# nanoporetech/remora

Hardware: AMD Instinct MI355X
Metric: chunks/sec, 5mC CG ConvLSTM_w_ref inference (fused chunk arrays -> logits + label counts) (higher is better)
Workload: dtype f32; 1 GPU; synthetic 100-sig-pt CG chunks, ConvLSTM_w_ref size 64 k-mer (4,4) 2-class (BASELINE configs[2]), fp32

## Files before the change

remora_amd/csrc/k_lstm.hip:

```cpp
#include "rmr_internal.h"
#include "rmr_math.h"
#include "rmr_mma.h"

namespace rmr {

struct LstmArgs {
    const float *x;
    float *logits;
    const float *a_ih1, *a_hh1, *b1, *a_ih2, *b2, *w_fc, *b_fc;
    int64_t n;
    int T, num_out;
};

template <int KS, int G, int RS>
__device__ __forceinline__ void xproj(const float (&buf)[4][16][RS], int q, int nn,
                                      const float (&A)[4][KS], f32x4 (&acc)[4]) {
    const float *b = &buf[q][nn][0];
#pragma unroll
    for (int g = 0; g < G; ++g) {
        const f32x4 bx = *reinterpret_cast<const f32x4 *>(b + 4 * g);
#pragma unroll
        for (int j = 0; j < 4; ++j)
#pragma unroll
            for (int gt = 0; gt < 4; ++gt)
                acc[gt] = __builtin_amdgcn_mfma_f32_16x16x4f32(A[gt][g * 4 + j], bx[j], acc[gt], 0, 0, 0);
    }
}

__device__ __forceinline__ float fc_dot4(const f32x4 wv, const f32x4 y) {
    return fmaf(wv[3], y[3], fmaf(wv[2], y[2], fmaf(wv[1], y[1], wv[0] * y[0])));
}

__device__ __forceinline__ void gates(const f32x4 (&acc)[4], f32x4 &c, f32x4 &h) {
#pragma unroll
    for (int r = 0; r < 4; ++r) {
        const float ig = sigmoid_f(acc[0][r]), fg = sigmoid_f(acc[1][r]);
        const float gg = tanh_f(acc[2][r]), og = sigmoid_f(acc[3][r]);
        c[r] = fg * c[r] + ig * gg;
        h[r] = og * tanh_f(c[r]);
    }
}

template <int H, bool HAS_H, bool HAS_X, int ABL>
__device__ __forceinline__ void lstm_step(const float (&xb_img)[4][16][(H / 16 % 2 == 0) ? H / 4 + 4 : H / 4],
                                          const float (&hb_img)[4][16][(H / 16 % 2 == 0) ? H / 4 + 4 : H / 4],
                                          int q, int nn, const float (&Aih)[4][H / 4], const float (&Ahh)[4][H / 4],
                                          const f32x4 (&bias)[4], f32x4 (&acc)[4], f32x4 (&accN)[4], f32x4 &c, f32x4 &h) {
    constexpr int KS = H / 4, G = H / 16;
    constexpr int RS = (G % 2 == 0) ? H / 4 + 4 : H / 4;
    f32x4 bx[G];
    if (HAS_X) {
        const float *xb = &xb_img[q][nn][0];
#pragma unroll
        for (int g = 0; g < G; ++g) bx[g] = *reinterpret_cast<const f32x4 *>(xb + 4 * g);
    }
    if (HAS_H) xproj<KS, G, RS>(hb_img, q, nn, Ahh, acc);
#pragma unroll
    for (int gt = 0; gt < 4; ++gt) accN[gt] = bias[gt];
    float ig[4], fg[4], gg[4];
#pragma unroll
    for (int s = 0; s < KS; ++s) {
        __builtin_amdgcn_sched_barrier(0);
        if (HAS_X) {
#pragma unroll
            for (int gt = 0; gt < 4; ++gt)
                accN[gt] = __builtin_amdgcn_mfma_f32_16x16x4f32(Aih[gt][s], bx[s >> 2][s & 3], accN[gt], 0, 0, 0);
        }
        for (int piece = s * 16 / KS; piece < (s + 1) * 16 / KS; ++piece) {
            const int r = piece >> 2, st = piece & 3;
            if (ABL & 1) {
                if (st == 3) { c[r] += acc[0][r] * acc[1][r]; h[r] = acc[2][r] + acc[3][r] * c[r]; }
                continue;
            }
            if (st == 0) ig[r] = fast_rcp(1.0f + __builtin_amdgcn_exp2f(acc[0][r]));
            if (st == 1) fg[r] = fast_rcp(1.0f + __builtin_amdgcn_exp2f(acc[1][r]));
            if (st == 2) {
                gg[r] = fmaf(-2.0f, fast_rcp(1.0f + __builtin_amdgcn_exp2f(acc[2][r])), 1.0f);
                c[r] = fmaf(fg[r], c[r], ig[r] * gg[r]);
            }
            if (st == 3) {
                const float og = fast_rcp(1.0f + __builtin_amdgcn_exp2f(acc[3][r]));
                h[r] = og * tanh_f(c[r]);
            }
        }
    }
    __builtin_amdgcn_sched_barrier(0);
}

template <int H, int ABL = 0>
__global__ __launch_bounds__(4 * H, 2) void lstm_head_kernel(LstmArgs a) {
    constexpr int NW = H / 16;
    constexpr int KS = H / 4;
    constexpr int G = H / 16;
    constexpr int RS = (G % 2 == 0) ? H / 4 + 4 : H / 4;
    static_assert((16 * RS) % 64 == 0, "plane must be a multiple of 64 floats");
    __shared__ __attribute__((aligned(16))) float xbuf[2][4][16][RS];
    __shared__ __attribute__((aligned(16))) float hbuf[2][4][16][RS];
    __shared__ float part[NW][16][16];
    extern __shared__ __attribute__((aligned(16))) float w2_lds[];

    const int tid = threadIdx.x;
    const int lane = tid & 63, w = tid >> 6, q = lane >> 4, nn = lane & 15;
    float *const w2 = w2_lds + (size_t)w * 3 * KS * 64 + lane;
    {
        const float *src = a.a_ih2 + (size_t)w * 3 * KS * 64 + lane;
#pragma unroll 8
        for (int i = 0; i < 3 * KS; ++i) w2[i * 64] = src[(size_t)i * 64];
    }

    float Aih[4][KS], Ahh[4][KS];
#pragma unroll
    for (int gt = 0; gt < 4; ++gt) {
        const float *pi = a.a_ih1 + ((size_t)(w * 4 + gt) * KS) * 64 + lane;
        const float *ph = a.a_hh1 + ((size_t)(w * 4 + gt) * KS) * 64 + lane;
#pragma unroll
        for (int s = 0; s < KS; ++s) {
            Aih[gt][s] = pi[(size_t)s * 64];
            Ahh[gt][s] = ph[(size_t)s * 64];
        }
    }
    f32x4 bias[4];
#pragma unroll
    for (int gt = 0; gt < 4; ++gt)
        bias[gt] = *reinterpret_cast<const f32x4 *>(a.b1 + gt * H + 16 * w + 4 * q);

    const int st_row = tid / (H / 4), st_c4 = tid - st_row * (H / 4);
    const int st_q = st_c4 & 3, st_g = st_c4 >> 2;

    const int64_t n_groups = (a.n + 15) / 16;
    for (int64_t grp = blockIdx.x; grp < n_groups; grp += gridDim.x) {
        const int64_t chunk0 = grp * 16;
        int64_t st_chunk = chunk0 + st_row;
        if (st_chunk >= a.n) st_chunk = a.n - 1;
        const float4 *xsrc = reinterpret_cast<const float4 *>(a.x + (size_t)st_chunk * a.T * H) + st_c4;
        RMR_SYNC();
        *reinterpret_cast<float4 *>(&xbuf[0][st_q][st_row][4 * st_g]) = xsrc[0];
        *reinterpret_cast<float4 *>(&xbuf[1][st_q][st_row][4 * st_g]) = xsrc[(size_t)(a.T > 1 ? 1 : 0) * (H / 4)];
        RMR_SYNC();

        f32x4 c = {0.f, 0.f, 0.f, 0.f};
        f32x4 accA[4] = {bias[0], bias[1], bias[2], bias[3]}, accB[4];
        xproj<KS, G, RS>(xbuf[0], q, nn, Aih, accA);
        RMR_SYNC();
#define RMR_LSTM_STEP(HAS_H, HAS_X, t_, p_, in, out)                                                                   \
    do {                                                                                                               \
        const int tt = (t_), pp = (p_);                                                                                \
        const int tf = (tt + 2 < a.T) ? tt + 2 : a.T - 1;                                                              \
        const float4 xnext = xsrc[(size_t)tf * (H / 4)];                                                               \
        f32x4 h;                                                                                                       \
        lstm_step<H, HAS_H, HAS_X, ABL>(xbuf[pp ^ 1], hbuf[pp ^ 1], q, nn, Aih, Ahh, bias, in, out, c, h);             \
        *reinterpret_cast<f32x4 *>(&hbuf[pp][q][nn][4 * w]) = h;                                                       \
        *reinterpret_cast<float4 *>(&xbuf[pp][st_q][st_row][4 * st_g]) = xnext;                                        \
        if (!(ABL & 2)) RMR_SYNC();                           \
    } while (0)
        RMR_LSTM_STEP(false, true, 0, 0, accA, accB);
        int t = 1;
        for (; t + 2 < a.T; t += 2) {
            RMR_LSTM_STEP(true, true, t, 1, accB, accA);
            RMR_LSTM_STEP(true, true, t + 1, 0, accA, accB);
        }
        if (t + 1 < a.T) {
            RMR_LSTM_STEP(true, true, t, 1, accB, accA);
#pragma unroll
            for (int gt = 0; gt < 4; ++gt) accB[gt] = accA[gt];
            ++t;
        }
        if (t < a.T) RMR_LSTM_STEP(true, false, t, t & 1, accB, accA);
#undef RMR_LSTM_STEP

        f32x4 acc2[3];
#pragma unroll
        for (int gt = 0; gt < 3; ++gt)
            acc2[gt] = *reinterpret_cast<const f32x4 *>(a.b2 + gt * H + 16 * w + 4 * q);
        {
            const float *hb = &hbuf[(a.T - 1) & 1][q][nn][0];
#pragma unroll
            for (int g = 0; g < G; ++g) {
                f32x4 z = *reinterpret_cast<const f32x4 *>(hb + 4 * g);
#pragma unroll
                for (int j = 0; j < 4; ++j) z[j] = swish_f(z[j]);
#pragma unroll
                for (int j = 0; j < 4; ++j)
#pragma unroll
                    for (int gt = 0; gt < 3; ++gt) {
                        const float aw = w2[(gt * KS + g * 4 + j) * 64];
                        acc2[gt] = __builtin_amdgcn_mfma_f32_16x16x4f32(aw, z[j], acc2[gt], 0, 0, 0);
                    }
            }
        }
        f32x4 y;
#pragma unroll
        for (int r = 0; r < 4; ++r) {
            const float c2 = sigmoid_f(acc2[0][r]) * tanh_f(acc2[1][r]);
            const float h2 = sigmoid_f(acc2[2][r]) * tanh_f(c2);
            y[r] = swish_f(h2);
        }
        for (int o = 0; o < a.num_out; ++o) {
            const f32x4 wv = *reinterpret_cast<const f32x4 *>(a.w_fc + (size_t)o * H + 16 * w + 4 * q);
            float p = fc_dot4(wv, y);
            p += __shfl_xor(p, 16);
            p += __shfl_xor(p, 32);
            if (q == 0) part[w][nn][o] = p;
        }
        RMR_SYNC();
#pragma unroll
        for (int i0 = 0; i0 < 16 * 16; i0 += 4 * H) {
            const int i = i0 + tid;
            if (i < 16 * a.num_out) {
                const int ch = i / a.num_out, o = i - ch * a.num_out;
                if (chunk0 + ch < a.n) {
                    float s = a.b_fc[o];
#pragma unroll
                    for (int ww = 0; ww < NW; ++ww) s += part[ww][ch][o];
                    a.logits[(size_t)(chunk0 + ch) * a.num_out + o] = s;
                }
            }
        }
    }
}

struct LstmSmallArgs {
    const float *x;
    float *logits;
    const float *s_ih1, *s_hh1, *s_ih2;
    const float *b1, *b2, *w_fc, *b_fc;
    int64_t n;
    int T, num_out;
};

template <bool HAS_H, bool HAS_X>
__device__ __forceinline__ void small_step(const float (&Ahh)[64], const float (&Aih)[64], const float *hrow, const float *xrow, f32x4 &acc,
                                           f32x4 &accN) {
#pragma unroll
    for (int g = 0; g < 4; ++g) {
        f32x4 hv[4], xv[4];
#pragma unroll
        for (int qq = 0; qq < 4; ++qq) {
            if (HAS_H) hv[qq] = *reinterpret_cast<const f32x4 *>(hrow + 16 * g + 4 * qq);
            if (HAS_X) xv[qq] = *reinterpret_cast<const f32x4 *>(xrow + 16 * g + 4 * qq);
        }
#pragma unroll
        for (int j = 0; j < 4; ++j)
#pragma unroll
            for (int qq = 0; qq < 4; ++qq) {
                if (HAS_H) acc = __builtin_amdgcn_mfma_f32_4x4x1f32(Ahh[(g * 4 + j) * 4 + qq], hv[qq][j], acc, 0, 0, 0);
                if (HAS_X) accN = __builtin_amdgcn_mfma_f32_4x4x1f32(Aih[(g * 4 + j) * 4 + qq], xv[qq][j], accN, 0, 0, 0);
            }
    }
}

__global__ __launch_bounds__(256, 1) void lstm_small_kernel(LstmSmallArgs a) {
    constexpr int H = 64;
    __shared__ __attribute__((aligned(16))) float xbuf[2][4][H + 4];
    __shared__ __attribute__((aligned(16))) float hbuf[2][4][H + 4];
    __shared__ __attribute__((aligned(16))) float ybuf[4][H + 4];
    const int tid = threadIdx.x, lane = tid & 63, w = tid >> 6;
    const int c = lane & 3, u = 16 * w + (lane >> 2);
    float Aih[H], Ahh[H];
#pragma unroll
    for (int p = 0; p < H; ++p) {
        Aih[p] = a.s_ih1[((size_t)w * H + p) * 64 + lane];
        Ahh[p] = a.s_hh1[((size_t)w * H + p) * 64 + lane];
    }
    const f32x4 bias = {a.b1[0 * H + u], a.b1[1 * H + u], a.b1[2 * H + u], a.b1[3 * H + u]};
    const f32x4 bias2 = {a.b2[0 * H + u], a.b2[1 * H + u], a.b2[2 * H + u], 0.0f};
    auto mm = [&](const float (&A)[H], const float *row, f32x4 acc, bool swish) {
#pragma unroll
        for (int g = 0; g < 4; ++g) {
            f32x4 v[4];
#pragma unroll
            for (int qq = 0; qq < 4; ++qq) {
                v[qq] = *reinterpret_cast<const f32x4 *>(row + 16 * g + 4 * qq);
                if (swish) {
#pragma unroll
                    for (int j = 0; j < 4; ++j) v[qq][j] = swish_f(v[qq][j]);
                }
            }
#pragma unroll
            for (int j = 0; j < 4; ++j)
#pragma unroll
                for (int qq = 0; qq < 4; ++qq)
                    acc = __builtin_amdgcn_mfma_f32_4x4x1f32(A[(g * 4 + j) * 4 + qq], v[qq][j], acc, 0, 0, 0);
        }
        return acc;
    };
    const int st_c = tid >> 6, st_k = tid & 63;
    const int64_t n_groups = (a.n + 3) / 4;
    for (int64_t grp = blockIdx.x; grp < n_groups; grp += gridDim.x) {
        const int64_t chunk0 = grp * 4;
        int64_t st_chunk = chunk0 + st_c;
        if (st_chunk >= a.n) st_chunk = a.n - 1;
        const float *xsrc = a.x + (size_t)st_chunk * a.T * H + st_k;
        RMR_SYNC();
        xbuf[0][st_c][st_k] = xsrc[0];
        xbuf[1][st_c][st_k] = xsrc[(size_t)(a.T > 1 ? 1 : 0) * H];
        RMR_SYNC();
        float cst = 0.0f;
        f32x4 accN = mm(Aih, &xbuf[0][c][0], bias, false);
        RMR_SYNC();
        for (int t = 0; t < a.T; ++t) {
            const float xnext = xsrc[(size_t)(t + 2 < a.T ? t + 2 : a.T - 1) * H];
            f32x4 acc = accN;
            accN = bias;
            const float *hrow = &hbuf[(t + 1) & 1][c][0], *xrow = &xbuf[(t + 1) & 1][c][0];
            if (t == 0) small_step<false, true>(Ahh, Aih, hrow, xrow, acc, accN);
            else if (t + 1 < a.T) small_step<true, true>(Ahh, Aih, hrow, xrow, acc, accN);
            else small_step<true, false>(Ahh, Aih, hrow, xrow, acc, accN);
            const float ig = fast_rcp(1.0f + __builtin_amdgcn_exp2f(acc[0]));
            const float fg = fast_rcp(1.0f + __builtin_amdgcn_exp2f(acc[1]));
            const float gg = fmaf(-2.0f, fast_rcp(1.0f + __builtin_amdgcn_exp2f(acc[2])), 1.0f);
            cst = fmaf(fg, cst, ig * gg);
            const float og = fast_rcp(1.0f + __builtin_amdgcn_exp2f(acc[3]));
            hbuf[t & 1][c][u] = og * tanh_f(cst);
            xbuf[t & 1][st_c][st_k] = xnext;
            RMR_SYNC();
        }
        float A2[H];
#pragma unroll
        for (int p = 0; p < H; ++p) A2[p] = a.s_ih2[((size_t)w * H + p) * 64 + lane];
        const f32x4 acc2 = mm(A2, &hbuf[(a.T - 1) & 1][c][0], bias2, true);
        const float c2 = sigmoid_f(acc2[0]) * tanh_f(acc2[1]);
        const float h2 = sigmoid_f(acc2[2]) * tanh_f(c2);
        ybuf[c][u] = swish_f(h2);
        RMR_SYNC();
        if (tid < 4 * a.num_out) {
            const int ch = tid / a.num_out, o = tid - ch * a.num_out;
            if (chunk0 + ch < a.n) {
                float s = a.b_fc[o];
                for (int ww = 0; ww < 4; ++ww) {
                    float pq[4];
                    for (int qq = 0; qq < 4; ++qq) {
                        const f32x4 wv = *reinterpret_cast<const f32x4 *>(a.w_fc + (size_t)o * H + 16 * ww + 4 * qq);
                        const f32x4 yv = *reinterpret_cast<const f32x4 *>(&ybuf[ch][16 * ww + 4 * qq]);
                        pq[qq] = fc_dot4(wv, yv);
                    }
                    s += (pq[0] + pq[1]) + (pq[2] + pq[3]);
                }
                a.logits[(size_t)(chunk0 + ch) * a.num_out + o] = s;
            }
        }
    }
}

static constexpr int64_t kLstmSmallMaxChunks = 1024;

template <int H>
static int launch_lstm_t(rmr_model *m, const float *x, int64_t n, float *logits) {
    rmr_engine *e = m->eng;
    LstmArgs a;
    a.x = x; a.logits = logits; a.n = n; a.T = m->T; a.num_out = m->desc.num_out;
    a.a_ih1 = m->lstm.a_ih1; a.a_hh1 = m->lstm.a_hh1; a.b1 = m->lstm.b1;
    a.a_ih2 = m->lstm.a_ih2; a.b2 = m->lstm.b2; a.w_fc = m->lstm.w_fc; a.b_fc = m->lstm.b_fc;
    const int64_t groups = (n + 15) / 16;
    int64_t grid = (int64_t)e->num_cus * 16;
    if (grid > groups) grid = groups;
    if (grid < 1) return 0;
    const size_t lds = (size_t)(H / 16) * 3 * (H / 4) * 64 * sizeof(float);
    RMR_TRY(e->allow_big_lds(reinterpret_cast<const void *>(lstm_head_kernel<H, 0>), lds));
    ProfScope ps(e, K_LSTM_HEAD);
#ifdef RMR_TIMING_ABLATIONS
    const int abl = abl_int("RMR_LSTM_ABLATE", 0);
    if (abl >= 1 && abl <= 3) {
        const void *k = abl == 1 ? reinterpret_cast<const void *>(lstm_head_kernel<H, 1>) : abl == 2 ? reinterpret_cast<const void *>(lstm_head_kernel<H, 2>) : reinterpret_cast<const void *>(lstm_head_kernel<H, 3>);
        RMR_TRY(e->allow_big_lds(k, lds));
    }
    if (abl == 1) hipLaunchKernelGGL((lstm_head_kernel<H, 1>), dim3((unsigned)grid), dim3(4 * H), lds, e->stream, a);
    else if (abl == 2) hipLaunchKernelGGL((lstm_head_kernel<H, 2>), dim3((unsigned)grid), dim3(4 * H), lds, e->stream, a);
    else if (abl == 3) hipLaunchKernelGGL((lstm_head_kernel<H, 3>), dim3((unsigned)grid), dim3(4 * H), lds, e->stream, a);
    else
#endif
    hipLaunchKernelGGL((lstm_head_kernel<H, 0>), dim3((unsigned)grid), dim3(4 * H), lds, e->stream, a);
    RMR_HIP(hipGetLastError());
    return 0;
}

int launch_lstm_head(rmr_model *m, const float *x, int64_t n, float *logits) {
    if (m->desc.size > 64) return launch_lstm_stream(m, x, n, logits);
    if (m->desc.size == 64 && n <= kLstmSmallMaxChunks && m->lstm.q_ih1) {
        rmr_engine *e = m->eng;
        LstmSmallArgs a;
        a.x = x; a.logits = logits; a.n = n; a.T = m->T; a.num_out = m->desc.num_out;
        a.s_ih1 = m->lstm.q_ih1; a.s_hh1 = m->lstm.q_hh1; a.s_ih2 = m->lstm.q_ih2;
        a.b1 = m->lstm.b1; a.b2 = m->lstm.b2; a.w_fc = m->lstm.w_fc; a.b_fc = m->lstm.b_fc;
        const int64_t groups = (n + 3) / 4;
        if (groups < 1) return 0;
        ProfScope ps(e, K_LSTM_HEAD);
        hipLaunchKernelGGL(lstm_small_kernel, dim3((unsigned)groups), dim3(256), 0, e->stream, a);
        RMR_HIP(hipGetLastError());
        return 0;
    }
    switch (m->desc.size) {
        case 64: return launch_lstm_t<64>(m, x, n, logits);
        case 32: return launch_lstm_t<32>(m, x, n, logits);
        case 16: return launch_lstm_t<16>(m, x, n, logits);
    }
    RMR_FAIL(RMR_ERR_INVALID, "unsupported LSTM size %d", m->desc.size);
}

__global__ __launch_bounds__(256) void fc_head_kernel(const float *m4, const float *w, const float *b, float *logits,
                                                      int64_t n, int size, int t4, int num_out) {
    const int lane = threadIdx.x & 63;
    const int64_t ch = (int64_t)blockIdx.x * 4 + (threadIdx.x >> 6);
    if (ch >= n) return;
    const float *src = m4 + (size_t)ch * t4 * size;
    const int total = t4 * size;
    float acc[16];
#pragma unroll
    for (int o = 0; o < 16; ++o) acc[o] = 0.0f;
    for (int e = lane; e < total; e += 64) {
        const float x = src[e];
        const int t = e / size, c = e - t * size;
        for (int o = 0; o < num_out; ++o) acc[o] += w[(size_t)o * total + c * t4 + t] * x;
    }
    for (int o = 0; o < num_out; ++o) {
        float v = acc[o];
        for (int s = 32; s > 0; s >>= 1) v += __shfl_xor(v, s);
        if (lane == 0) logits[ch * num_out + o] = v + b[o];
    }
}

int launch_fc_head(rmr_model *m, const float *m4, int64_t n, float *logits) {
    rmr_engine *e = m->eng;
    const int64_t total = n * m->desc.num_out;
    if (total == 0) return 0;
    ProfScope ps(e, K_FC_HEAD);
    hipLaunchKernelGGL(fc_head_kernel, dim3((unsigned)((n + 3) / 4)), dim3(256), 0, e->stream,
                       m4, m->w_fc, m->b_fc, logits, n, m->desc.size, m->T4, m->desc.num_out);
    RMR_HIP(hipGetLastError());
    return 0;
}

}
```

Before: 31.59 million chunks/s.

## Overlap LSTM x-projection tail with recurrent step and prefetch next chunk group

Result: no change. 31.74 million chunks/s (median of 6 runs) (+0.5%).

```diff
diff --git a/remora_amd/csrc/k_lstm.hip b/remora_amd/csrc/k_lstm.hip
--- a/remora_amd/csrc/k_lstm.hip
+++ b/remora_amd/csrc/k_lstm.hip
@@ -41,32 +41,62 @@
     }
 }
 
+template <int H>
+struct LstmHeld {
+    static constexpr int KS = H / 4;
+    static constexpr int R = 4 <= KS / 2 ? 4 : KS / 2;
+    static_assert(R % 2 == 0 && R <= 4, "held slices: 2 or 4");
+};
+
+template <int H, int FIRST>
+__device__ __forceinline__ void x_tail(const float (&Aih)[4][H / 4], const f32x4 xt, f32x4 (&acc)[4]) {
+    constexpr int KS = H / 4, R = LstmHeld<H>::R;
+#pragma unroll
+    for (int s = KS - R + FIRST; s < KS - R + FIRST + R / 2; ++s)
+#pragma unroll
+        for (int gt = 0; gt < 4; ++gt) acc[gt] = __builtin_amdgcn_mfma_f32_16x16x4f32(Aih[gt][s], xt[s & 3], acc[gt], 0, 0, 0);
+}
+
 template <int H, bool HAS_H, bool HAS_X, int ABL>
 __device__ __forceinline__ void lstm_step(const float (&xb_img)[4][16][(H / 16 % 2 == 0) ? H / 4 + 4 : H / 4],
                                           const float (&hb_img)[4][16][(H / 16 % 2 == 0) ? H / 4 + 4 : H / 4],
                                           int q, int nn, const float (&Aih)[4][H / 4], const float (&Ahh)[4][H / 4],
-                                          const f32x4 (&bias)[4], f32x4 (&acc)[4], f32x4 (&accN)[4], f32x4 &c, f32x4 &h) {
-    constexpr int KS = H / 4, G = H / 16;
-    constexpr int RS = (G % 2 == 0) ? H / 4 + 4 : H / 4;
-    f32x4 bx[G];
+                                          const f32x4 (&bias)[4], f32x4 (&acc)[4], f32x4 (&accN)[4], f32x4 &c, f32x4 &h, f32x4 &xt) {
+    constexpr int KS = H / 4, G = H / 16, R = LstmHeld<H>::R, KG = KS - R;
+    f32x4 bx[G], bh[G];
+    if (HAS_H) {
+        const float *hb = &hb_img[q][nn][0];
+#pragma unroll
+        for (int g = 0; g < G; ++g) bh[g] = *reinterpret_cast<const f32x4 *>(hb + 4 * g);
+    }
     if (HAS_X) {
         const float *xb = &xb_img[q][nn][0];
 #pragma unroll
         for (int g = 0; g < G; ++g) bx[g] = *reinterpret_cast<const f32x4 *>(xb + 4 * g);
     }
-    if (HAS_H) xproj<KS, G, RS>(hb_img, q, nn, Ahh, acc);
+    if (HAS_H) {
+        __builtin_amdgcn_sched_barrier(0);
+        x_tail<H, R / 2>(Aih, xt, acc);
+        __builtin_amdgcn_sched_barrier(0);
+#pragma unroll
+        for (int s = 0; s < KS; ++s)
+#pragma unroll
+            for (int gt = 0; gt < 4; ++gt)
+                acc[gt] = __builtin_amdgcn_mfma_f32_16x16x4f32(Ahh[gt][s], bh[s >> 2][s & 3], acc[gt], 0, 0, 0);
+    }
+    if (HAS_X) xt = bx[G - 1];
 #pragma unroll
     for (int gt = 0; gt < 4; ++gt) accN[gt] = bias[gt];
     float ig[4], fg[4], gg[4];
 #pragma unroll
-    for (int s = 0; s < KS; ++s) {
+    for (int s = 0; s < KG; ++s) {
         __builtin_amdgcn_sched_barrier(0);
         if (HAS_X) {
 #pragma unroll
             for (int gt = 0; gt < 4; ++gt)
                 accN[gt] = __builtin_amdgcn_mfma_f32_16x16x4f32(Aih[gt][s], bx[s >> 2][s & 3], accN[gt], 0, 0, 0);
         }
-        for (int piece = s * 16 / KS; piece < (s + 1) * 16 / KS; ++piece) {
+        for (int piece = s * 16 / KG; piece < (s + 1) * 16 / KG; ++piece) {
             const int r = piece >> 2, st = piece & 3;
             if (ABL & 1) {
                 if (st == 3) { c[r] += acc[0][r] * acc[1][r]; h[r] = acc[2][r] + acc[3][r] * c[r]; }
@@ -128,29 +158,51 @@
     const int st_q = st_c4 & 3, st_g = st_c4 >> 2;
 
     const int64_t n_groups = (a.n + 15) / 16;
+    const bool handoff = (a.T & 1) == 0 && a.T >= 2;
+    bool staged = false;
+    f32x4 accA[4], accB[4];
     for (int64_t grp = blockIdx.x; grp < n_groups; grp += gridDim.x) {
         const int64_t chunk0 = grp * 16;
         int64_t st_chunk = chunk0 + st_row;
         if (st_chunk >= a.n) st_chunk = a.n - 1;
         const float4 *xsrc = reinterpret_cast<const float4 *>(a.x + (size_t)st_chunk * a.T * H) + st_c4;
-        RMR_SYNC();
-        *reinterpret_cast<float4 *>(&xbuf[0][st_q][st_row][4 * st_g]) = xsrc[0];
-        *reinterpret_cast<float4 *>(&xbuf[1][st_q][st_row][4 * st_g]) = xsrc[(size_t)(a.T > 1 ? 1 : 0) * (H / 4)];
-        RMR_SYNC();
-
-        f32x4 c = {0.f, 0.f, 0.f, 0.f};
-        f32x4 accA[4] = {bias[0], bias[1], bias[2], bias[3]}, accB[4];
-        xproj<KS, G, RS>(xbuf[0], q, nn, Aih, accA);
+        const bool next_staged = handoff && grp + gridDim.x < n_groups;
+        const float4 *xwrap = xsrc + (size_t)(a.T - 1) * (H / 4);
+        size_t wrap_stride = 0;
+        if (next_staged) {
+            int64_t nx_chunk = chunk0 + (int64_t)gridDim.x * 16 + st_row;
+            if (nx_chunk >= a.n) nx_chunk = a.n - 1;
+            xwrap = reinterpret_cast<const float4 *>(a.x + (size_t)nx_chunk * a.T * H) + st_c4;
+            wrap_stride = H / 4;
+        }
+        if (!staged) {
+            RMR_SYNC();
+            *reinterpret_cast<float4 *>(&xbuf[0][st_q][st_row][4 * st_g]) = xsrc[0];
+            *reinterpret_cast<float4 *>(&xbuf[1][st_q][st_row][4 * st_g]) = xsrc[(size_t)(a.T > 1 ? 1 : 0) * (H / 4)];
+            RMR_SYNC();
+        }
+
+        f32x4 c = {0.f, 0.f, 0.f, 0.f}, xt = {0.f, 0.f, 0.f, 0.f};
+        if (!staged) {
+#pragma unroll
+            for (int gt = 0; gt < 4; ++gt) accA[gt] = bias[gt];
+            xproj<KS, G, RS>(xbuf[0], q, nn, Aih, accA);
+        }
+        staged = next_staged;
         RMR_SYNC();
 #define RMR_LSTM_STEP(HAS_H, HAS_X, t_, p_, in, out)                                                                   \
     do {                                                                                                               \
         const int tt = (t_), pp = (p_);                                                                                \
-        const int tf = (tt + 2 < a.T) ? tt + 2 : a.T - 1;                                                              \
-        const float4 xnext = xsrc[(size_t)tf * (H / 4)];                                                               \
+        const float4 xnext = (tt + 2 < a.T) ? xsrc[(size_t)(tt + 2) * (H / 4)] : xwrap[(size_t)(tt + 2 - a.T) * wrap_stride]; \
         f32x4 h;                                                                                                       \
-        lstm_step<H, HAS_H, HAS_X, ABL>(xbuf[pp ^ 1], hbuf[pp ^ 1], q, nn, Aih, Ahh, bias, in, out, c, h);             \
+        lstm_step<H, HAS_H, HAS_X, ABL>(xbuf[pp ^ 1], hbuf[pp ^ 1], q, nn, Aih, Ahh, bias, in, out, c, h, xt);         \
         *reinterpret_cast<f32x4 *>(&hbuf[pp][q][nn][4 * w]) = h;                                                       \
         *reinterpret_cast<float4 *>(&xbuf[pp][st_q][st_row][4 * st_g]) = xnext;                                        \
+        if (HAS_X) {                               \
+            __builtin_amdgcn_sched_barrier(0);                                                                         \
+            x_tail<H, 0>(Aih, xt, out);                                                                                \
+            __builtin_amdgcn_sched_barrier(0);                                                                         \
+        }                                                                                                              \
         if (!(ABL & 2)) RMR_SYNC();                           \
     } while (0)
         RMR_LSTM_STEP(false, true, 0, 0, accA, accB);
@@ -187,6 +239,11 @@
                         acc2[gt] = __builtin_amdgcn_mfma_f32_16x16x4f32(aw, z[j], acc2[gt], 0, 0, 0);
                     }
             }
+        }
+        if (staged) {
+#pragma unroll
+            for (int gt = 0; gt < 4; ++gt) accA[gt] = bias[gt];
+            xproj<KS, G, RS>(xbuf[0], q, nn, Aih, accA);
         }
         f32x4 y;
 #pragma unroll
@@ -344,6 +401,8 @@
 
 static constexpr int64_t kLstmSmallMaxChunks = 1024;
 
+static constexpr int kLstmBlocksPerCU = 16;
+
 template <int H>
 static int launch_lstm_t(rmr_model *m, const float *x, int64_t n, float *logits) {
     rmr_engine *e = m->eng;
@@ -352,7 +411,7 @@
     a.a_ih1 = m->lstm.a_ih1; a.a_hh1 = m->lstm.a_hh1; a.b1 = m->lstm.b1;
     a.a_ih2 = m->lstm.a_ih2; a.b2 = m->lstm.b2; a.w_fc = m->lstm.w_fc; a.b_fc = m->lstm.b_fc;
     const int64_t groups = (n + 15) / 16;
-    int64_t grid = (int64_t)e->num_cus * 16;
+    int64_t grid = (int64_t)e->num_cus * kLstmBlocksPerCU;
     if (grid > groups) grid = groups;
     if (grid < 1) return 0;
     const size_t lds = (size_t)(H / 16) * 3 * (H / 4) * 64 * sizeof(float);
```
